# TrevorS/voxtral-mini-realtime-rs

Measured on NVIDIA H100. Metric: decode_tokens_per_sec, higher is better.
Workload: dtype f32

## Files before the change

voxtral_mini_realtime_rs_b200/csrc/capi.cu:

```cuda
#include <cuda_profiler_api.h>
#include <cuda_runtime.h>

#include <cstring>
#include <memory>
#include <string>
#include <vector>

#include "audio_host.h"
#include "common.h"
#include "gguf.h"
#include "kernels.h"
#include "model.h"
#include "stream.h"
#include "tokenizer.h"

namespace vox {
static thread_local std::string g_last_error;
void set_last_error(const std::string &m) { g_last_error = m; }
}

using namespace vox;

#define VOX_API_BEGIN try {
#define VOX_API_END                                \
// ... 882 lines not shown
    VOX_API_END
}
int32_t vox_session_nbest(vox_session *sh, int32_t *ids, double *scores, size_t cap, int32_t *b, int32_t *w, int32_t *n) {
    VOX_API_BEGIN
    REQUIRE(sh);
    Session *s = sh->s;
    s->sel.read_nbest(ids, scores, cap, b, w, n, s->st);
    VOX_API_END
}
int32_t vox_session_cache_len(const vox_session *s, int32_t *len) {
    VOX_API_BEGIN
    REQUIRE(s); REQUIRE(len);
    *len = s->s->cache_len;
    VOX_API_END
}
int32_t vox_session_reset(vox_session *s) {
    VOX_API_BEGIN
    REQUIRE(s);
    CUDA_OK(cudaSetDevice(s->s->m->device));
    s->s->reset();
    CUDA_OK(cudaStreamSynchronize(s->s->st));
    VOX_API_END
}
int32_t vox_session_debug_read(vox_session *sh, const char *what, float *out, size_t cap, size_t *n_floats) {
    VOX_API_BEGIN
    REQUIRE(sh); REQUIRE(what);
    Session *s = sh->s;
    const vox_model_info &c = s->m->info;
    CUDA_OK(cudaSetDevice(s->m->device));
    const std::string w = what;
    const float *src = nullptr;
    size_t n = 0;
    AudioEncoder &e = s->enc;
    const size_t rows = (size_t)e.rows;
    if (w == "capture_on" || w == "capture_off") {
        e.set_capture(*s, w == "capture_on");
        if (n_floats) *n_floats = 0;
        return VOX_OK;
    } else if (w == "graph_off" || w == "graph_on") {
        s->use_graph = (w == "graph_on");
        if (n_floats) *n_floats = 0;
        return VOX_OK;
    } else if (w == "enc_attn_simt" || w == "enc_attn_tc") {
        e.use_attn_tc = (w == "enc_attn_tc");
        if (n_floats) *n_floats = 0;
        return VOX_OK;
    } else if (w == "gemm_simt" || w == "gemm_tc") {
        s->path.gemm_tc = (w == "gemm_tc");
        if (n_floats) *n_floats = 0;
        return VOX_OK;
    } else if (w == "mega_off" || w == "mega_on" || w == "mega_auto") {
        s->use_mega = (w != "mega_off");
        if (n_floats) *n_floats = 0;
        return VOX_OK;
    } else if (w == "tc_off" || w == "tc_on") {
        s->path.matvec_tc = (w == "tc_on");
        if (n_floats) *n_floats = 0;
        return VOX_OK;
    } else if (w == "mega_epoch") {
        int epoch = 0;
        CUDA_OK(cudaStreamSynchronize(s->st));
        CUDA_OK(cudaMemcpy(&epoch, s->mega.epoch, sizeof(int), cudaMemcpyDeviceToHost));
        const float v[2] = {(float)s->mega.launches, (float)epoch};
        if (n_floats) *n_floats = 2;
        if (out) {
            VOX_CHECK(cap >= 2, VOX_ECAPACITY, "debug_read capacity %zu < 2", cap);
            memcpy(out, v, sizeof(v));
        }
        return VOX_OK;
    } else if (w == "mega_attn") {
        const size_t cnt = s->mega.attn_log.size() * 4;
        if (n_floats) *n_floats = cnt;
        if (out) {
            VOX_CHECK(cap >= cnt, VOX_ECAPACITY, "debug_read capacity %zu < %zu", cap, cnt);
            for (size_t i = 0; i < cnt; ++i) out[i] = (float)s->mega.attn_log[i / 4][i % 4];
        }
        return VOX_OK;
    } else if ((w.rfind("kv_k", 0) == 0 || w.rfind("kv_v", 0) == 0) && w.size() > 4) {
        const int l = atoi(w.c_str() + 4);
        VOX_CHECK(l >= 0 && l < c.dec_layers && std::to_string(l) == w.substr(4), VOX_EINVAL, "no decoder layer in '%s'", what);
        const int B = s->cur_B;
        std::vector<int> pos(B);
        CUDA_OK(cudaStreamSynchronize(s->st));
        if (B) CUDA_OK(cudaMemcpy(pos.data(), s->d_pos, sizeof(int) * B, cudaMemcpyDeviceToHost));
        const int L = B ? std::min(pos[0], s->kv.capacity()) : 0;
        for (int b = 0; b < B; ++b) VOX_CHECK(pos[b] == pos[0], VOX_EINVAL, "'%s': rows at different positions", what);
        const size_t cnt = (size_t)B * L * c.dec_kv_heads * c.dec_head_dim;
        if (n_floats) *n_floats = cnt;
        if (out && cnt) {
            VOX_CHECK(cap >= cnt, VOX_ECAPACITY, "debug_read capacity %zu < %zu", cap, cnt);
            s->kv.read(l, w[3] == 'v', B, L, out);
        }
        return VOX_OK;
    } else if (w == "mega_trace") {
        const size_t cnt = (size_t)s->mega.n_ops * 6;
        if (n_floats) *n_floats = cnt;
        if (out) {
            VOX_CHECK(cap >= cnt, VOX_ECAPACITY, "debug_read capacity %zu < %zu", cap, cnt);
            CUDA_OK(cudaStreamSynchronize(s->st));
            std::vector<unsigned long long> t(cnt);
            if (cnt) CUDA_OK(cudaMemcpy(t.data(), s->mega.trace, sizeof(unsigned long long) * cnt, cudaMemcpyDeviceToHost));
            int khz = 0;
            CUDA_OK(cudaDeviceGetAttribute(&khz, cudaDevAttrClockRate, s->m->device));
            for (size_t i = 0; i < cnt; ++i) out[i] = (float)((double)(t[i] - t[0]) / ((double)khz * 1e-3));
        }
        return VOX_OK;
// ... 299 lines not shown
```

voxtral_mini_realtime_rs_b200/csrc/decode_mega.cu:

```cuda
#include <cuda_fp16.h>

#include <cfloat>
#include <cmath>
#include <cstdlib>

#include "common.h"
#include "model.h"

namespace vox {

enum MegaKind : int {
    MG_EMBED = 0,
    MG_MATVEC = 1,
    MG_ATTN = 2,
    MG_ARGMAX = 3,
};

struct MegaOp {
    int kind = 0, epi = 0;
    const uint4 *qs_tc = nullptr;
    const uint2 *d_tc = nullptr;
    int N = 0, K = 0, n_tiles = 0, n_pairs = 0;
    int S = 1, Ps = 0;
    const uint2 *fin_bf = nullptr;
// ... 102 lines not shown
__host__ __device__ constexpr int mg_attn_fixed_bytes(int G, int HD) { return (G * HD + MG_CWARPS * G) * 4; }
__host__ __device__ constexpr int mg_attn_key_bytes(int G, int HD, KvType t) {
    return t == KvType::Q8 ? G * 4 + (2 * HD + 16) + 2 * (HD / KV_Q8_BLOCK) * 2
                           : G * 4 + (2 * HD + 16 / (t == KvType::F16 ? 2 : 4)) * (t == KvType::F16 ? 2 : 4);
}
__host__ __device__ constexpr int mg_attn_tile(int scratch_bytes, int G, int HD, KvType t) {
    return (scratch_bytes - mg_attn_fixed_bytes(G, HD)) / mg_attn_key_bytes(G, HD, t) / 32 * 32 > MG_CTHREADS
               ? MG_CTHREADS
               : (scratch_bytes - mg_attn_fixed_bytes(G, HD)) / mg_attn_key_bytes(G, HD, t) / 32 * 32;
}

__device__ __forceinline__ uint32_t smem_u32(const void *p) { return (uint32_t)__cvta_generic_to_shared(p); }
__device__ __forceinline__ void mbar_init(uint64_t *bar, uint32_t count) {
    asm volatile("mbarrier.init.shared::cta.b64 [%0], %1;\n" ::"r"(smem_u32(bar)), "r"(count));
}
__device__ __forceinline__ void mbar_expect_tx(uint64_t *bar, uint32_t bytes) {
    asm volatile("mbarrier.arrive.expect_tx.shared::cta.b64 _, [%0], %1;\n" ::"r"(smem_u32(bar)), "r"(bytes) : "memory");
}
__device__ __forceinline__ void mbar_arrive(uint64_t *bar) {
    asm volatile("mbarrier.arrive.shared::cta.b64 _, [%0];\n" ::"r"(smem_u32(bar)) : "memory");
}
__device__ __forceinline__ bool mbar_try(uint64_t *bar, uint32_t parity) {
    uint32_t ok;
    asm volatile(
        "{\n"
        ".reg .pred p;\n"
        "mbarrier.try_wait.parity.shared::cta.b64 p, [%1], %2;\n"
        "selp.u32 %0, 1, 0, p;\n"
        "}\n"
        : "=r"(ok)
        : "r"(smem_u32(bar)), "r"(parity)
        : "memory");
    return ok != 0;
}
__device__ __noinline__ void mg_die(unsigned *flag, unsigned code) {
    atomicExch(flag, code);
    __threadfence_system();
    __trap();
}
__device__ __forceinline__ void mbar_wait(uint64_t *bar, uint32_t parity, unsigned *flag, unsigned code) {
    if (mbar_try(bar, parity)) return;
    const long long t0 = clock64();
    unsigned n = 0;
    while (!mbar_try(bar, parity)) {
        if ((++n & 0x3FFFu) == 0 && clock64() - t0 > MG_SPIN_CYCLES) mg_die(flag, code);
    }
}
__device__ __forceinline__ void bulk_g2s(void *dst_smem, const void *src_gmem, uint32_t bytes, uint64_t *bar) {
    asm volatile("cp.async.bulk.shared::cluster.global.mbarrier::complete_tx::bytes [%0], [%1], %2, [%3];\n" ::"r"(
                     smem_u32(dst_smem)),
                 "l"(src_gmem), "r"(bytes), "r"(smem_u32(bar))
                 : "memory");
}
__device__ __forceinline__ unsigned ld_relaxed_u32(const unsigned *p) {
    unsigned v;
    asm volatile("ld.relaxed.gpu.global.u32 %0, [%1];\n" : "=r"(v) : "l"(p) : "memory");
    return v;
}
__device__ __forceinline__ void st_tagged(float2 *p, const float v, const int tag) {
    asm volatile("st.relaxed.gpu.global.v2.f32 [%0], {%1, %2};\n" ::"l"(p), "f"(v), "f"(__int_as_float(tag)) : "memory");
}
__device__ __forceinline__ float2 ld_tagged(const float2 *p) {
    float2 v;
    asm volatile("ld.relaxed.gpu.global.v2.f32 {%0, %1}, [%2];\n" : "=f"(v.x), "=f"(v.y) : "l"(p) : "memory");
    return v;
}
__device__ __forceinline__ void red_release_add(unsigned *p, unsigned v) {
    asm volatile("red.release.gpu.global.add.u32 [%0], %1;\n" ::"l"(p), "r"(v) : "memory");
}
__device__ __forceinline__ void cp_async16(void *dst_smem, const void *src_gmem) {
    asm volatile("cp.async.cg.shared.global [%0], [%1], 16;\n" ::"r"(smem_u32(dst_smem)), "l"(src_gmem) : "memory");
}
__device__ __forceinline__ void cp_async_commit() { asm volatile("cp.async.commit_group;\n" ::: "memory"); }
template <int N>
__device__ __forceinline__ void cp_async_wait() { asm volatile("cp.async.wait_group %0;\n" ::"n"(N) : "memory"); }
__device__ __forceinline__ void prefetch_l1(const void *p) { asm volatile("prefetch.global.L1 [%0];\n" ::"l"(p)); }
__device__ __forceinline__ void bulk_prefetch_l2(const void *p, uint32_t bytes) {
    asm volatile("cp.async.bulk.prefetch.L2.global [%0], %1;\n" ::"l"(p), "r"(bytes) : "memory");
}
__device__ __forceinline__ uint64_t policy_evict_first() {
    uint64_t pol;
    asm volatile("createpolicy.fractional.L2::evict_first.b64 %0, 1.0;\n" : "=l"(pol));
    return pol;
}
__device__ __forceinline__ void bulk_g2s_hint(void *dst_smem, const void *src_gmem, uint32_t bytes, uint64_t *bar, uint64_t pol) {
    asm volatile(
        "cp.async.bulk.shared::cluster.global.mbarrier::complete_tx::bytes.L2::cache_hint [%0], [%1], %2, [%3], %4;\n" ::"r"(
            smem_u32(dst_smem)),
        "l"(src_gmem), "r"(bytes), "r"(smem_u32(bar)), "l"(pol)
        : "memory");
}
__device__ __forceinline__ void cbar() { asm volatile("bar.sync 1, 512;\n" ::: "memory"); }
__device__ __forceinline__ void ebar() { asm volatile("bar.sync 2, %0;\n" ::"n"(MG_ETHREADS) : "memory"); }
__device__ __forceinline__ void abar() { asm volatile("bar.sync 3, %0;\n" ::"n"(MG_ATHREADS) : "memory"); }
__device__ __forceinline__ void hbar_arrive(const int id, const bool publish) {
    if (publish) asm volatile("fence.acq_rel.cta;\n" ::: "memory");
    asm volatile("bar.arrive %0, %1;\n" ::"r"(id), "n"(MG_ATHREADS) : "memory");
}
__device__ __forceinline__ void hbar_sync(const int id) { asm volatile("bar.sync %0, %1;\n" ::"r"(id), "n"(MG_ATHREADS) : "memory"); }

__device__ __forceinline__ void mma16816(float (&c)[4], const uint32_t a0, const uint32_t a1, const uint32_t a2,
                                         const uint32_t a3, const uint32_t b0, const uint32_t b1) {
    asm volatile(
        "mma.sync.aligned.m16n8k16.row.col.f32.f16.f16.f32 {%0,%1,%2,%3}, {%4,%5,%6,%7}, {%8,%9}, {%0,%1,%2,%3};\n"
        : "+f"(c[0]), "+f"(c[1]), "+f"(c[2]), "+f"(c[3])
        : "r"(a0), "r"(a1), "r"(a2), "r"(a3), "r"(b0), "r"(b1));
// ... 117 lines not shown
                blo[c] = make_uint2(0u, 0u);
                bhi[c] = blo[c];
                if (col < 2 * MT) {
                    blo[c] = bfb[col * 4 + t];
                    bhi[c] = bfb[(2 * MT + col) * 4 + t];
                }
                const int tok = c * 4 + t;
                of[c] = tok < MT ? ofp[bb * MT + tok] : make_float2(0.0f, 0.0f);
            }
#pragma unroll
            for (int u = 0; u < NTV; ++u) {
                const uint32_t wg = bb ? wq[u].z : wq[u].x, wg8 = bb ? wq[u].w : wq[u].y;
                const uint32_t dw = bb ? wd[u].y : wd[u].x;
                const float2 d = __half22float2(*reinterpret_cast<const __half2 *>(&dw));
                const uint32_t sg = wg >> 8, sg8 = wg8 >> 8;
#pragma unroll
                for (int c = 0; c < CG; ++c) {
                    float cc[4] = {0.f, 0.f, 0.f, 0.f};
                    mma16816(cc, wg & 0x000F000Fu, wg8 & 0x000F000Fu, sg & 0x000F000Fu, sg8 & 0x000F000Fu, blo[c].x, blo[c].y);
                    mma16816(cc, wg & 0x00F000F0u, wg8 & 0x00F000F0u, sg & 0x00F000F0u, sg8 & 0x00F000F0u, bhi[c].x, bhi[c].y);
                    acc[u][2 * c] = fmaf(d.x, fmaf(cc[0] + cc[1], of[c].y, of[c].x), acc[u][2 * c]);
                    acc[u][2 * c + 1] = fmaf(d.y, fmaf(cc[2] + cc[3], of[c].y, of[c].x), acc[u][2 * c + 1]);
                }
            }
        }
    }
}

template <int MT, int G, int DPL, bool RING, typename KV>
__global__ void __launch_bounds__(MG_THREADS, 1) decode_mega_kernel(const MegaParams p) {
    constexpr int CG = (MT + 3) / 4;
    constexpr int HD = DPL * 32;
    static_assert(G * HD <= MG_CTHREADS, "one attention output per consumer thread");
    constexpr int NT = mg_nt(MT);
    extern __shared__ __align__(128) unsigned char smem[];
    uint64_t *full = reinterpret_cast<uint64_t *>(smem);
    uint64_t *empty = full + MG_MAX_STAGES;
    float *rinv = reinterpret_cast<float *>(empty + MG_MAX_STAGES + 2);
    float *rpart = rinv + 8;
    uint64_t *stgc = reinterpret_cast<uint64_t *>(rpart + 32);
    float *red = reinterpret_cast<float *>(stgc + 4);
    float *acc_tile = red + 2 * MG_CWARPS * NT * 16 * MT;
    float *vals = acc_tile + MG_ACC_TILES * 16 * MT;
    MegaOp *s_op = reinterpret_cast<MegaOp *>(vals + mg_vals(MT));
    static_assert(sizeof(MegaOp) <= 256 && sizeof(MegaOp) % 4 == 0, "s_op");
    uint64_t *stg = empty + MG_MAX_STAGES;
    unsigned char *scratch = smem + mg_misc_bytes(MT);
    unsigned char *ring = scratch + p.scratch_bytes;
    const int tid = threadIdx.x, warp = tid >> 5, lane = tid & 31;
    const int g = lane >> 2, t = lane & 3;
    const int cta = blockIdx.x, nctas = gridDim.x;
    const int B = p.B, nstage = p.nstage;
    unsigned *wd_flag = p.bar + 2;

    if (tid == 0) {
        for (int i = 0; i < nstage; ++i) {
            mbar_init(&full[i], 1);
            mbar_init(&empty[i], MG_CWARPS);
        }
        mbar_init(stg, 1);
        for (int c = 0; c < 4; ++c) mbar_init(&stgc[c], 1);
        asm volatile("fence.mbarrier_init.release.cluster;\n" ::: "memory");
    }
    __syncthreads();

    if (warp >= MG_CWARPS) {
        asm volatile("setmaxnreg.dec.sync.aligned.u32 %0;\n" ::"n"(MG_REGS_PRODUCER));
        if (warp == MG_CWARPS && lane == 0) {
            int stage = 0;
            uint32_t phase = 0;
            bool wrapped = false;
            const uint64_t pol = policy_evict_first();
            for (int oi = 0; oi < p.n_ops; ++oi) {
                const MegaOp &op = p.ops[oi];
                if (oi + 1 < p.n_ops) {
                    const MegaOp &nx = p.ops[oi + 1];
                    const int who = (cta - oi % nctas + nctas) % nctas;
                    if (nx.kind == MG_MATVEC) {
                        if (nx.fout_ada_layer >= 0) {
                            if (who < B) bulk_prefetch_l2(p.ffn_ada_rows[who] + (size_t)nx.fout_ada_layer * p.D, (uint32_t)nx.N * 4u);
                        } else if (who == 0 && nx.fout_gamma) {
                            bulk_prefetch_l2(nx.fout_gamma, (uint32_t)nx.N * 4u);
                        }
                    }
                }
                if (op.kind != MG_MATVEC) continue;
                const int n_tiles = op.n_tiles, n_pairs = op.n_pairs, S = op.S, Ps = op.Ps, UT = op.unit_tiles;
                const uint4 *qs = op.qs_tc;
                const uint2 *ds = op.d_tc;
                const int ntl = mg_tile_count(n_tiles, UT, cta, nctas);
                for (int s = 0; s < S; ++s) {
                    const int pb = s * Ps;
                    const int np = min(Ps, n_pairs - pb);
                    for (int it = 0; it < ntl; it += NT) {
                        const int nt = min(NT, ntl - it);
                        for (int c0 = 0; c0 < np; c0 += MG_CHUNK) {
                            const int nb = min(MG_CHUNK, np - c0);
                            if (wrapped) mbar_wait(&empty[stage], phase ^ 1u, wd_flag, 0x100u + (unsigned)oi);
                            unsigned char *dst = ring + (size_t)stage * (NT * MG_SLOT_BYTES);
                            mbar_expect_tx(&full[stage], (uint32_t)(nt * nb) * 576u);
                            for (int u = 0; u < nt; ++u) {
                                const size_t pair0 = (size_t)mg_tile_of(it + u, UT, cta, nctas) * n_pairs + pb + c0;
                                bulk_g2s_hint(dst + (size_t)u * MG_SLOT_BYTES, qs + pair0 * 32, (uint32_t)nb * 512u, &full[stage], pol);
                                bulk_g2s_hint(dst + (size_t)u * MG_SLOT_BYTES + MG_SLOT_Q, ds + pair0 * 8, (uint32_t)nb * 64u, &full[stage], pol);
                            }
                            if (++stage == nstage) {
                                stage = 0;
                                phase ^= 1u;
                                wrapped = true;
                            }
                        }
                    }
                }
            }
        } else if (warp > MG_CWARPS) {
            constexpr int NOUT = NT * 16 * MT;
            constexpr int NQ = NOUT / 4;
// ... 290 lines not shown
                }
                if (oi + 1 < p.n_ops) {
                    abar();
                    abar();
                }
            }
        }
        return;
    }

    asm volatile("setmaxnreg.inc.sync.aligned.u32 %0;\n" ::"n"(MG_REGS_CONSUMER));
    const int epoch = *p.d_epoch;
    int stage = 0;
    uint32_t phase = 0, stg_phase = 0;
    int par = 0, group_ctr = 0;
    unsigned bar_target = 0;

    for (int oi = 0; oi < p.n_ops; ++oi) {
        const MegaOp &op = p.ops[oi];
        const int kind = op.kind;
        const bool tracing = p.trace != nullptr && cta == 0 && tid == 0;
        const bool tr_all = p.trace_all != nullptr && tid == 0;
        unsigned long long *const ta = tr_all ? p.trace_all + ((size_t)cta * p.n_ops + oi) * 4 : nullptr;
        if (tr_all) ta[0] = ta[3] = (unsigned long long)clock64();
        if (tracing) {
            const unsigned long long now = (unsigned long long)clock64();
            p.trace[oi * 6 + 0] = now;
            p.trace[oi * 6 + 1] = now;
            p.trace[oi * 6 + 4] = now;
            p.trace[oi * 6 + 5] = now;
        }
        if (tid == 0 && oi + 1 < p.n_ops) {
            prefetch_l1(&p.ops[oi + 1]);
            prefetch_l1(reinterpret_cast<const unsigned char *>(&p.ops[oi + 1]) + 128);
        }
        if (kind == MG_MATVEC) {
            const int n_tiles = op.n_tiles, n_pairs = op.n_pairs, S = op.S, Ps = op.Ps, K = op.K;
            const int UT = op.unit_tiles;
            const bool has_norm = op.gamma != nullptr;
            const int ntl = mg_tile_count(n_tiles, UT, cta, nctas);
            float2 *off2 = reinterpret_cast<float2 *>(scratch);
            uint2 *bf = reinterpret_cast<uint2 *>(off2 + (size_t)Ps * 2 * MT);
            if (ntl > 0) {
                for (int s = 0; s < S; ++s) {
                    const int pb = s * Ps;
                    const int np = min(Ps, n_pairs - pb);
                    const int CP = 16 * ((((np + 15) >> 4) + 3) >> 2);
                    cbar();
                    if (tid == 0) {
                        asm volatile("fence.proxy.async;\n" ::: "memory");
                        const uint32_t ob = (uint32_t)(2 * np * MT) * 8u;
                        const unsigned char *src = reinterpret_cast<const unsigned char *>(op.fin_bf + (size_t)(2 * pb) * (16 * MT));
                        unsigned char *dstb = reinterpret_cast<unsigned char *>(bf);
#pragma unroll
                        for (int c = 0; c < 4; ++c) {
                            const int p0 = min(np, c * CP), p1 = min(np, (c + 1) * CP);
                            const uint32_t o = (uint32_t)p0 * (256u * MT), cb = (uint32_t)(p1 - p0) * (256u * MT);
                            mbar_expect_tx(&stgc[c], cb + (c == 0 ? ob : 0u));
                            if (c == 0) bulk_g2s(off2, op.fin_off + (size_t)(2 * pb) * MT, ob, &stgc[0]);
                            if (cb) bulk_g2s(dstb + o, src + o, cb, &stgc[c]);
                        }
                    }
                    const uint32_t stg_par = stg_phase;
                    stg_phase ^= 1u;
                    if (s == 0 && has_norm && warp >= 1 && warp <= 4) {
                        const int total = op.ssq_in_parts * 8;
                        float pr[12];
#pragma unroll
                        for (int q = 0; q < 12; ++q) {
                            const int f = (warp - 1) * 32 + lane + 128 * q;
                            pr[q] = f < total ? __ldcg(op.ssq_in + f) : 0.0f;
                        }
                        float ss = 0.0f;
#pragma unroll
                        for (int q = 0; q < 12; ++q) ss += pr[q];
                        for (int f = (warp - 1) * 32 + lane + 128 * 12; f < total; f += 128) ss += __ldcg(op.ssq_in + f);
                        ss += __shfl_xor_sync(0xffffffffu, ss, 8);
                        ss += __shfl_xor_sync(0xffffffffu, ss, 16);
                        if (lane < 8) rpart[(warp - 1) * 8 + lane] = ss;
                    }
                    cbar();
                    if (s == 0 && has_norm && tid < B)
                        rinv[tid] = 1.0f / sqrtf((((rpart[tid] + rpart[8 + tid]) + (rpart[16 + tid] + rpart[24 + tid]))) / (float)K + p.eps);
                    if (tracing && s == 0) p.trace[oi * 6 + 1] = (unsigned long long)clock64();
                    for (int it = 0; it < ntl; it += NT) {
                        const int nt = min(NT, ntl - it);
                        float acc[NT][2 * CG];
#pragma unroll
                        for (int u = 0; u < NT; ++u)
#pragma unroll
                            for (int c = 0; c < 2 * CG; ++c) acc[u][c] = 0.0f;
                        {
                            const uint32_t slot_q = (uint32_t)warp * 512u + (uint32_t)lane * 16u;
                            const uint32_t slot_d = (uint32_t)MG_SLOT_Q + (uint32_t)warp * 64u + (uint32_t)g * 8u;
                            int next_chunk_c0 = it == 0 ? 0 : 0x7fffffff, chunk = 0;
                            for (int c0 = 0; c0 < np; c0 += MG_CHUNK) {
                                if (c0 == next_chunk_c0) {
                                    mbar_wait(&stgc[chunk], stg_par, wd_flag, 0x500u + (unsigned)oi);
                                    ++chunk;
                                    next_chunk_c0 += CP;
                                }
                                mbar_wait(&full[stage], phase, wd_flag, 0x200u + (unsigned)oi);
                                if (tracing && s == 0 && it == 0 && c0 == 0) p.trace[oi * 6 + 4] = (unsigned long long)clock64();
                                if (tr_all && s == 0 && it == 0 && c0 == 0) ta[3] = (unsigned long long)clock64();
                                const int pp = c0 + warp;
                                if (pp < np) {
                                    const unsigned char *sb = ring + (size_t)stage * (NT * MG_SLOT_BYTES);
                                    const uint2 *bfp = bf + (size_t)pp * (2 * 16 * MT);
                                    const float2 *ofp = off2 + (size_t)pp * (2 * MT);
                                    uint64_t *const rel = &empty[stage];
                                    if (nt == NT) mg_pair<MT, NT, NT>(sb, slot_q, slot_d, bfp, ofp, g, t, lane, acc, rel);
                                    else if (NT > 1 && nt == 1) mg_pair<MT, NT, 1>(sb, slot_q, slot_d, bfp, ofp, g, t, lane, acc, rel);
                                    else if (NT > 2 && nt == 2) mg_pair<MT, NT, 2>(sb, slot_q, slot_d, bfp, ofp, g, t, lane, acc, rel);
// ... 354 lines not shown
                if (warp < B) {
                    float bv = -INFINITY;
                    int bx = 0x7fffffff;
                    for (int c = lane; c < nctas; c += 32)
                        amax_combine(bv, bx, __ldcg(p.am_vals + (size_t)c * 8 + warp), __ldcg(p.am_idx + (size_t)c * 8 + warp));
#pragma unroll
                    for (int o = 16; o > 0; o >>= 1) {
                        const float ov = __shfl_xor_sync(0xffffffffu, bv, o);
                        const int ox = __shfl_xor_sync(0xffffffffu, bx, o);
                        amax_combine(bv, bx, ov, ox);
                    }
                    if (lane == 0) {
                        if (bx == 0x7fffffff) bx = 0;
                        p.d_tok[warp] = bx;
                        const int outpos = p.d_outpos[warp];
                        if (p.d_out) p.d_out[(size_t)warp * p.out_ld + outpos] = bx;
                        p.d_pos[warp] += 1;
                        p.d_outpos[warp] = outpos + 1;
                    }
                }
                if (tid == 0) *p.d_epoch = epoch + 1;
            }
        }
        if (tracing) p.trace[oi * 6 + 2] = (unsigned long long)clock64();
        if (tr_all) ta[1] = ta[2] = (unsigned long long)clock64();
        if (oi + 1 < p.n_ops) {
            abar();
            if (tid == 0) {
                red_release_add(&p.bar[0], 1u);
                bar_target += (unsigned)nctas;
                const long long t0 = clock64();
                unsigned n = 0;
                while (ld_relaxed_u32(&p.bar[0]) < bar_target) {
                    if ((++n & 0x3FFu) == 0 && clock64() - t0 > MG_SPIN_CYCLES) mg_die(wd_flag, 0x300u + (unsigned)oi);
                }
                asm volatile("fence.acq_rel.gpu;\n" ::: "memory");
            }
            abar();
            if (tracing) p.trace[oi * 6 + 3] = (unsigned long long)clock64();
            if (tr_all) ta[2] = (unsigned long long)clock64();
        }
    }
    if (tid == 0) {
        __threadfence();
        const unsigned old = atomicAdd(&p.bar[1], 1u);
        if (old == (unsigned)nctas - 1u) {
            p.bar[0] = 0u;
            p.bar[1] = 0u;
            __threadfence();
        }
    }
}

template <int MT, int G, int DPL, bool RING, typename KV>
void launch_t(const MegaParams &p, const MegaPlan &plan, int grid, cudaStream_t st) {
    static SmemAttr smem_attr;
    CUDA_OK(ensure_dyn_smem(decode_mega_kernel<MT, G, DPL, RING, KV>, MG_SMEM_MAX, smem_attr));
    cudaLaunchConfig_t cfg{};
    cfg.gridDim = dim3(grid);
    cfg.blockDim = dim3(MG_THREADS);
    cfg.dynamicSmemBytes = plan.smem_bytes;
    cfg.stream = st;
    cudaLaunchAttribute attr[1];
    attr[0].id = cudaLaunchAttributeCooperative;
    attr[0].val.cooperative = 1;
    cfg.attrs = attr;
    cfg.numAttrs = 1;
    CUDA_OK(cudaLaunchKernelEx(&cfg, decode_mega_kernel<MT, G, DPL, RING, KV>, p));
    tc_count_launch("decode_mega");
}

template <int MT, int G, int DPL>
void launch_g(const MegaParams &p, const MegaPlan &plan, int grid, cudaStream_t st) {
    if (plan.kv_type == KvType::Q8) (p.ring ? launch_t<MT, G, DPL, true, int8_t> : launch_t<MT, G, DPL, false, int8_t>)(p, plan, grid, st);
    else if (plan.kv_type == KvType::F16) (p.ring ? launch_t<MT, G, DPL, true, __half> : launch_t<MT, G, DPL, false, __half>)(p, plan, grid, st);
    else (p.ring ? launch_t<MT, G, DPL, true, float> : launch_t<MT, G, DPL, false, float>)(p, plan, grid, st);
}


using MegaLaunch = void (*)(const MegaParams &, const MegaPlan &, int, cudaStream_t);
template <int G, int DPL>
MegaLaunch mt_launch(int MT) {
    return MT == 1 ? launch_g<1, G, DPL> : MT == 2 ? launch_g<2, G, DPL> : MT == 4 ? launch_g<4, G, DPL>
                                                                             : launch_g<8, G, DPL>;
}
MegaLaunch find_launch(int MT, int H, int Hkv, int hd) {
    const int G = Hkv > 0 && H % Hkv == 0 ? H / Hkv : 0;
    if (G == 4 && hd == 128) return mt_launch<4, 4>(MT);
    if (G == 2 && hd == 32) return mt_launch<2, 1>(MT);
    return nullptr;
}

MegaPlan decode_mega_plan(int B, int max_pairs, int H, int Hkv, int hd, KvType kv_type) {
    MegaPlan pl;
    pl.kv_type = kv_type;
    pl.MT = B <= 1 ? 1 : (B <= 2 ? 2 : (B <= 4 ? 4 : 8));
    const int G = H / Hkv;
    const int attn_bytes = mg_attn_fixed_bytes(G, hd) + 32 * mg_attn_key_bytes(G, hd, kv_type);
    const int per_pair = mg_pair_bytes(pl.MT);
    int cap_pairs = MG_SCRATCH_CAP / per_pair;
    if (cap_pairs >= MG_CHUNK) cap_pairs = cap_pairs / MG_CHUNK * MG_CHUNK;
    pl.Ps_cap = max_pairs < cap_pairs ? max_pairs : cap_pairs;
    if (pl.Ps_cap < 1) pl.Ps_cap = 1;
    int scratch = pl.Ps_cap * per_pair;
    if (scratch < attn_bytes) scratch = attn_bytes;
    pl.scratch_bytes = (scratch + 127) & ~127;
    pl.attn_tile = mg_attn_tile(pl.scratch_bytes, G, hd, kv_type);
    const int left = MG_SMEM_MAX - mg_misc_bytes(pl.MT) - pl.scratch_bytes;
    const int stage_bytes = mg_nt(pl.MT) * MG_SLOT_BYTES;
    int ns = left / stage_bytes;
    pl.nstage = ns > MG_MAX_STAGES ? MG_MAX_STAGES : ns;
    VOX_CHECK(pl.nstage >= 2, VOX_EINVAL, "decode_mega: no room for the weight ring (%d stages)", pl.nstage);
    pl.smem_bytes = (size_t)mg_misc_bytes(pl.MT) + pl.scratch_bytes + (size_t)pl.nstage * stage_bytes;
    return pl;
}

}

struct MegaFrag {
    uint2 *bf = nullptr;
    float2 *off = nullptr;
    size_t blocks = 0;
};

struct DecodeMega::State {
    MegaParams p;
    MegaPlan plan;
    MegaOp *ops = nullptr;
    int ops_cap = 0;
    int rows = 0;
    int att_units = 0;
    size_t acc_floats = 0, ml_floats = 0;
    MegaFrag xf, af, cf;
    void clear_fragments(cudaStream_t st) const {
        for (const MegaFrag *f : {&xf, &af, &cf}) CUDA_OK(cudaMemsetAsync(f->bf, 0, sizeof(uint2) * f->blocks * 16 * MG_ROWS, st));
        for (const MegaFrag *f : {&xf, &af, &cf}) CUDA_OK(cudaMemsetAsync(f->off, 0, sizeof(float2) * f->blocks * MG_ROWS, st));
    }
};

DecodeMega::DecodeMega() : state(new State) {}
DecodeMega::~DecodeMega() = default;

void DecodeMega::create(Session &s) {
    const Model &m = *s.m;
    const vox_model_info &c = m.info;
    State &g = *state;
    MegaParams &p = g.p;
    CUDA_OK(cudaDeviceGetAttribute(&grid, cudaDevAttrMultiProcessorCount, m.device));
    g.ops_cap = 6 * c.dec_layers + 4;
    p.ops = g.ops = s.arena.alloc_n<MegaOp>(g.ops_cap);
    p.bar = s.arena.alloc_n<unsigned>(4);
    CUDA_OK(cudaMemset(p.bar, 0, sizeof(unsigned) * 4));
    p.am_vals = s.arena.alloc_n<float>((size_t)grid * MG_ROWS);
    p.am_idx = s.arena.alloc_n<int>((size_t)grid * MG_ROWS);
    g.att_units = std::max(grid, MG_ROWS * c.dec_kv_heads);
    const size_t units = g.att_units + MG_ROWS * c.dec_kv_heads, G = c.dec_heads / c.dec_kv_heads;
    g.acc_floats = 2 * units * G * c.dec_head_dim;
    g.ml_floats = 2 * units * G * 2;
    p.att_acc = s.arena.alloc_n<float>(g.acc_floats);
    p.att_ml = s.arena.alloc_n<float>(g.ml_floats);
    p.d_epoch = epoch = s.arena.alloc_n<int>(1);
    CUDA_OK(cudaMemset(p.att_acc, 0, sizeof(float) * g.acc_floats));
    CUDA_OK(cudaMemset(p.att_ml, 0, sizeof(float) * g.ml_floats));
    CUDA_OK(cudaMemset(epoch, 0, sizeof(int)));
    g.xf.blocks = 2 * mg_pairs(c.dec_dim);
    g.af.blocks = 2 * mg_pairs(c.dec_heads * c.dec_head_dim);
    g.cf.blocks = 2 * mg_pairs(c.dec_ffn);
    for (MegaFrag *f : {&g.xf, &g.af, &g.cf}) f->bf = s.arena.alloc_n<uint2>(f->blocks * 16 * MG_ROWS);
    for (MegaFrag *f : {&g.xf, &g.af, &g.cf}) f->off = s.arena.alloc_n<float2>(f->blocks * MG_ROWS);
    p.trace = trace = s.arena.alloc_n<unsigned long long>((size_t)g.ops_cap * 6);
    CUDA_OK(cudaMemset(trace, 0, sizeof(unsigned long long) * g.ops_cap * 6));
    if (const char *ta = getenv("VOX_MEGA_TRACE_ALL"); ta && ta[0] == '1') {
        const size_t n = (size_t)grid * g.ops_cap * 4;
        p.trace_all = trace_all = s.arena.alloc_n<unsigned long long>(n);
        CUDA_OK(cudaMemset(trace_all, 0, sizeof(unsigned long long) * n));
    }
    p.eps = m.norm_eps;
    p.qkv = s.qkv_dec;
    p.ld_qkv = (c.dec_heads + 2 * c.dec_kv_heads) * c.dec_head_dim;
    p.H = c.dec_heads;
    p.Hkv = c.dec_kv_heads;
    p.hd = c.dec_head_dim;
    const KvView kv = s.kv.view(0, s.d_pos);
    p.max_seq = kv.max_seq();
    p.page_table = kv.page_table;
    p.max_pages = kv.max_pages;
    p.window = c.dec_window;
    p.scale = powf((float)c.dec_head_dim, -0.5f);
    p.ring = kv.ring ? 1 : 0;
    p.attn_out = s.attn_dec;
    p.emb_qs = m.tok_emb.qs;
    p.emb_d = m.tok_emb.d;
    p.D = c.dec_dim;
    p.audio_off = s.d_audio_off;
    p.ffn_ada_rows = s.d_fga_rows;
    p.x_dec = s.x_dec;
    p.ssq_x = s.ssq_x;
    p.emb_fbf = g.xf.bf;
    p.emb_foff = g.xf.off;
    p.emb_gamma = m.dec[0].attn_norm;
    p.att_fbf = g.af.bf;
    p.att_foff = g.af.off;
    p.d_pos = s.d_pos;
    p.d_outpos = s.d_outpos;
    p.d_tok = s.d_tok;
    p.d_out = s.d_out;
    p.out_ld = s.out_ld;
}

unsigned DecodeMega::prepare(const Session &s, int R) {
    const Model &m = *s.m;
    const vox_model_info &c = m.info;
    State &g = *state;
    const int B = std::min(R, MG_ROWS);
    const unsigned groups = (unsigned)(R + MG_ROWS - 1) / MG_ROWS;
    const int D = c.dec_dim, H = c.dec_heads, Hkv = c.dec_kv_heads, hd = c.dec_head_dim;
    if (B < 1 || !find_launch(1, H, Hkv, hd)) return 0;
    if (g.rows == B) return n_ops > 0 ? groups : 0;
    g.rows = B;
    n_ops = 0;
    for (int j = 0; j < c.dec_layers; ++j)
        if (!m.dec[j].wqkv.qs_tc || !m.dec[j].wo.qs_tc || !m.dec[j].w13.qs_tc || !m.dec[j].w2.qs_tc) return 0;
    const int max_pairs = std::max(std::max(mg_pairs(D), mg_pairs(H * hd)), mg_pairs(c.dec_ffn));
    g.plan = decode_mega_plan(B, max_pairs, H, Hkv, hd, s.kv.type());
    const int parts = (D + 15) / 16;
    std::vector<MegaOp> ops;
    bool ok = true;
    auto matvec = [&](const Q4Weight &w, const MegaFrag &fin, float *y, int ldy, const float *res, int epi, const float *norm_w,
                      bool ssq_out_, bool track, int unit_tiles, const MegaFrag &fout, const float *fout_gamma) {
        MegaOp o;
        o.kind = MG_MATVEC;
        o.epi = epi;
        o.qs_tc = w.qs_tc;
        o.d_tc = w.d_tc;
        o.N = w.N;
        o.K = w.K;
        o.n_tiles = (w.N + 15) / 16;
        o.n_pairs = mg_pairs(w.K);
        int S = (o.n_pairs + g.plan.Ps_cap - 1) / g.plan.Ps_cap;
        int Ps = (o.n_pairs + S - 1) / S;
        if (S > 1) Ps = std::min(g.plan.Ps_cap, (Ps + 15) / 16 * 16);
        S = (o.n_pairs + Ps - 1) / Ps;
        o.S = S;
        o.Ps = Ps;
        o.unit_tiles = unit_tiles;
        if (o.n_tiles % unit_tiles != 0) ok = false;
        const int n_units = o.n_tiles / unit_tiles;
        if (S > 1 && ((n_units + grid - 1) / grid) * unit_tiles > MG_ACC_TILES) ok = false;
        o.fin_bf = fin.bf;
        o.fin_off = fin.off;
        o.fout_bf = fout.bf;
        o.fout_off = fout.off;
        o.fout_gamma = fout_gamma;
        o.y = y;
        o.ldy = ldy;
        o.res = res;
        o.gamma = norm_w;
        if (norm_w) {
            o.ssq_in = s.ssq_x;
            o.ssq_in_parts = parts;
        }
        if (ssq_out_) o.ssq_out = s.ssq_x;
        o.track_argmax = track ? 1 : 0;
        ops.push_back(o);
    };
    const MegaFrag none;
    {
        MegaOp e;
        e.kind = MG_EMBED;
        ops.push_back(e);
    }
    for (int j = 0; j < c.dec_layers; ++j) {
        const DecLayerW &l = m.dec[j];
        matvec(l.wqkv, g.xf, s.qkv_dec, g.p.ld_qkv, nullptr, EPI_NONE, l.attn_norm, false, false, 1, none, nullptr);
        const KvView kv = s.kv.view(j, s.d_pos);
        ops.back().kc = kv.k;
        ops.back().vc = kv.v;
        MegaOp a;
        a.kind = MG_ATTN;
        a.kc = kv.k;
        a.vc = kv.v;
        a.layer = j;
        ops.push_back(a);
        matvec(l.wo, g.af, s.x_dec, D, s.x_dec, EPI_RESIDUAL, nullptr, true, false, 2, g.xf, nullptr);
        ops.back().fout_ada_layer = j;
        matvec(l.w13, g.xf, nullptr, c.dec_ffn, nullptr, EPI_SILU_MUL, l.ffn_norm, false, false, 4, g.cf, nullptr);
        const float *next_norm = j + 1 < c.dec_layers ? m.dec[j + 1].attn_norm : m.dec_norm;
        matvec(l.w2, g.cf, s.x_dec, D, s.x_dec, EPI_RESIDUAL, nullptr, true, false, 2, g.xf, next_norm);
    }
    matvec(m.tok_emb, g.xf, s.logits, c.vocab, nullptr, EPI_NONE, m.dec_norm, false, true, 1, none, nullptr);
    {
        MegaOp f;
        f.kind = MG_ARGMAX;
        ops.push_back(f);
    }
    if (c.dec_ffn % 32 != 0 || (H * hd) % 32 != 0 || c.dec_layers > 63) ok = false;
    if ((D + 15) / 16 != parts || D % 32 != 0) ok = false;
    if (!ok || (int)ops.size() > g.ops_cap) return 0;
    g.clear_fragments(s.st);
    CUDA_OK(cudaMemcpyAsync(g.ops, ops.data(), sizeof(MegaOp) * ops.size(), cudaMemcpyHostToDevice, s.st));
    CUDA_OK(cudaStreamSynchronize(s.st));
    n_ops = g.p.n_ops = (int)ops.size();
    return groups;
}

void DecodeMega::step(const Session &s, int R, bool add_audio) {
    const State &g = *state;
    for (int b0 = 0; b0 < R; b0 += MG_ROWS) {
        const int B = std::min(MG_ROWS, R - b0);
        if (B < g.rows) {
            g.clear_fragments(s.st);
        }
        MegaParams p = g.p;
        p.B = B;
        p.page_table += (size_t)b0 * p.max_pages;
        p.audio_off += b0;
        p.ffn_ada_rows += b0;
        p.d_pos += b0;
        p.d_outpos += b0;
        p.d_tok += b0;
        p.d_out += (size_t)b0 * p.out_ld;
        p.audio = add_audio ? s.enc.audio : nullptr;
        p.logits_out = s.logits + (size_t)b0 * s.m->info.vocab;
        p.cos_t = s.dec_rope.cos_t;
        p.sin_t = s.dec_rope.sin_t;
        p.rope_rows = s.dec_rope.rows;
        p.attn_chunks = std::max(1, std::min(4, std::min(grid, g.att_units) / (B * p.Hkv)));
        p.nstage = g.plan.nstage;
        p.scratch_bytes = g.plan.scratch_bytes;
        attn_log.push_back({B, g.plan.MT, g.plan.attn_tile, p.attn_chunks});
        find_launch(g.plan.MT, p.H, p.Hkv, p.hd)(p, g.plan, grid, s.st);
        if (!capturing) ++launches;
    }
}

void DecodeMega::rebase_epoch(cudaStream_t st) {
    if (launches > (1u << 24)) {
        CUDA_OK(cudaMemsetAsync(state->p.att_acc, 0, sizeof(float) * state->acc_floats, st));
        CUDA_OK(cudaMemsetAsync(state->p.att_ml, 0, sizeof(float) * state->ml_floats, st));
        CUDA_OK(cudaMemsetAsync(epoch, 0, sizeof(int), st));
        launches = 0;
    }
}

}
```

voxtral_mini_realtime_rs_b200/csrc/decode_mega.h:

```cpp
#pragma once
#include <cuda_runtime.h>

#include <array>
#include <memory>
#include <vector>

namespace vox {

struct Session;

struct DecodeMega {
    DecodeMega();
    ~DecodeMega();
    void create(Session &s);
    unsigned prepare(const Session &s, int R);
    void step(const Session &s, int R, bool add_audio);
    void rebase_epoch(cudaStream_t st);

    unsigned launches = 0;
    bool capturing = false;
    std::vector<std::array<int, 4>> attn_log;
    int grid = 0, n_ops = 0;
    int *epoch = nullptr;
    unsigned long long *trace = nullptr, *trace_all = nullptr;

  private:
    struct State;
    std::unique_ptr<State> state;
};

}
```

voxtral_mini_realtime_rs_b200/csrc/model.cu:

```cuda
#include "model.h"

#include <algorithm>
#include <cmath>
#include <cstring>

#include "common.h"

namespace vox {

void cuda_check(cudaError_t e, const char *what) {
    if (e != cudaSuccess) fail(VOX_ECUDA, fmt("CUDA error: %s: %s", what, cudaGetErrorString(e)));
}

void *DeviceArena::alloc(size_t bytes) {
    if (bytes == 0) bytes = 16;
    void *p = nullptr;
    cudaError_t e = cudaMalloc(&p, bytes);
    if (e != cudaSuccess) fail(VOX_ENOMEM, fmt("cudaMalloc(%zu) failed: %s", bytes, cudaGetErrorString(e)));
    ptrs.push_back(p);
    total += bytes;
    return p;
}

void DeviceArena::release() {
// ... 597 lines not shown
                     fused_decode(B) ? ssq_x : nullptr, st);
        const bool pending = decoder_forward(B, 1);
        lm_head_rows(B, pending, logits);
        launch_argmax_multi(logits, B, m->info.vocab, d_tok, d_out, out_ld, d_outpos, am_vals, am_idx, am_cnt, st);
        launch_advance(d_pos, 1, d_outpos, 1, B, st);
    }
    sel.after_step(*this, B);
    return mega_launches;
}

void Session::set_bias(int stream, const int32_t *ids, const int32_t *lens, const float *boosts, int n) {
    if (sel.set_bias(stream, ids, lens, boosts, n, st)) bound_streams.clear();
}

void Session::prefill(int B, int M, const int *ids_host, bool add_audio) {
    const vox_model_info &c = m->info;
    bind_rows(B);
    CUDA_OK(cudaMemcpyAsync(d_ids, ids_host, sizeof(int) * (size_t)B * M, cudaMemcpyHostToDevice, st));
    launch_embed(m->tok_emb, d_ids, add_audio ? enc.audio : nullptr, d_audio_off, B, M, d_pos, x_dec,
                 fused_decode(B * M) ? ssq_x : nullptr, st);
    const bool pending = decoder_forward(B, M);
    if (pending) {
        launch_rmsnorm(x_dec, m->dec_norm, h_dec, B * M, c.dec_dim, m->norm_eps, st);
    }
    launch_gather_last(h_dec, last_h, B, M, c.dec_dim, st);
    linear(m->tok_emb, last_h, B, logits, c.vocab, nullptr, nullptr, EPI_NONE);
    launch_argmax(logits, B, c.vocab, d_tok, d_out, out_ld, d_outpos, st);
    launch_advance(d_pos, M, d_outpos, 1, B, st);
    sel.after_step(*this, B);
}

void Session::step_incremental(int b, int M, const int *ids_host, bool add_audio) {
    if (ids_host) prefill(b, M, ids_host, add_audio);
    else decode_step(b, add_audio);
    cache_len += M;
    sel.record_step(b, out_rows.data());
    for (int r = 0; r < b; ++r) ++out_rows[r];
}

void Session::reset() {
    CUDA_OK(cudaMemsetAsync(d_pos, 0, sizeof(int) * max_batch, st));
    CUDA_OK(cudaMemsetAsync(d_outpos, 0, sizeof(int) * max_batch, st));
    std::fill(out_rows.begin(), out_rows.end(), 0);
    cache_len = 0;
    kv.restore_identity(st);
    sel.clear_bias_history(-1, st);
    rebase_epoch();
}

template <class Step>
void Session::run_steps(int R, int n, Step step) {
    if (n <= 0) return;
    prepare_step(R);
    const StepKey key{R, sel.top_k, sel.beam_w, path.matvec_tc, path.gemm_tc, use_mega, sel.bias_on()};
    if (use_graph && !(step_graph.exec && step_graph.key == key)) {
        step();
        --n;
        if (step_graph.exec) { cudaGraphExecDestroy(step_graph.exec); step_graph.exec = nullptr; }
        if (n > 0) {
            cudaGraph_t graph = nullptr;
            const uint64_t before = kernel_launch_count();
            CUDA_OK(cudaStreamBeginCapture(st, cudaStreamCaptureModeThreadLocal));
            mega.capturing = true;
            try {
                step_graph.mega_launches = step();
            } catch (...) {
                mega.capturing = false;
                cudaStreamEndCapture(st, &graph);
                if (graph) cudaGraphDestroy(graph);
                throw;
            }
            mega.capturing = false;
            CUDA_OK(cudaStreamEndCapture(st, &graph));
            step_graph.nodes = kernel_launch_count() - before;
            add_graph_launches(-(int64_t)step_graph.nodes);
            cudaError_t e = cudaGraphInstantiate(&step_graph.exec, graph, 0);
            cudaGraphDestroy(graph);
            cuda_check(e, "cudaGraphInstantiate");
            step_graph.key = key;
        }
    }
    for (int i = 0; i < n; ++i) {
        if (!use_graph) { step(); continue; }
        CUDA_OK(cudaGraphLaunch(step_graph.exec, st));
        add_graph_launches((int64_t)step_graph.nodes);
        mega.launches += step_graph.mega_launches;
    }
}

namespace {
struct RowStreams {
    Session *s;
    ~RowStreams() { s->row_streams.clear(); }
};
}

int Session::transcribe_from_mel(int B, int T, int32_t *out_ids, size_t cap_ids, vox_timings *tm, bool total) {
    const vox_model_info &c = m->info;
    const int W = sel.beam_w, R = B * W;
    sel.check_rows(B);
    RowStreams row_guard{this};
    if (W > 1)
        for (int r = 0; r < R; ++r) row_streams.push_back(r % B);
    const std::vector<int> frames(B, T);
    enc.encode(*this, B, frames.data());
    cur_B = B;
    CUDA_OK(cudaEventRecord(ev[2], st));
// ... 143 lines not shown
```

voxtral_mini_realtime_rs_b200/csrc/model.h:

```cpp
#pragma once
#include <cuda_runtime.h>

#include <algorithm>
#include <cstdint>
#include <string>
#include <tuple>
#include <vector>

#include "audio_host.h"
#include "gguf.h"
#include "decode_mega.h"
#include "encoder.h"
#include "kernels.h"
#include "kv_cache.h"
#include "token_select.h"

namespace vox {

void cuda_check(cudaError_t e, const char *what);
#define CUDA_OK(x) ::vox::cuda_check((x), #x)

struct DeviceArena {
    int device = 0;
    std::vector<void *> ptrs;
// ... 15 lines not shown
void alloc_split_k(DeviceArena &arena, Work &w) {
    w.partial = arena.alloc_n<float>(w.partial_floats);
    w.counters = arena.alloc_n<int>(w.n_counters);
    CUDA_OK(cudaMemset(w.counters, 0, sizeof(int) * w.n_counters));
}

struct MelTables {
    float *window = nullptr;
    float *fb_vals = nullptr;
    int *fb_start = nullptr, *fb_len = nullptr;
    int fb_stride = 0;
    std::vector<float> fb_dense, window_host;
    void build(DeviceArena &arena);
};

struct EncLayerW {
    float *attn_norm = nullptr, *ffn_norm = nullptr;
    Q4Weight wqkv, wo, w13, w2;
    float *bqkv = nullptr, *bo = nullptr, *b2 = nullptr;
};
struct DecLayerW {
    float *attn_norm = nullptr, *ffn_norm = nullptr;
    Q4Weight ada0, ada2, wqkv, wo, w13, w2;
};

struct Model {
    int device = 0;
    vox_model_info info{};
    float rope_theta = 1e6f, norm_eps = 1e-5f;
    DeviceArena arena;
    float *conv1_w = nullptr, *conv1_b = nullptr, *conv2_w = nullptr, *conv2_b = nullptr;
    std::vector<EncLayerW> enc;
    float *enc_norm = nullptr;
    Q4Weight adapter0, adapter2, tok_emb;
    std::vector<DecLayerW> dec;
    float *dec_norm = nullptr;
    float *enc_cos = nullptr, *enc_sin = nullptr, *dec_cos = nullptr, *dec_sin = nullptr;
    int enc_rope_len = 4096, dec_rope_len = 16384;
    MelTables mel;
    RopeView dec_rope() const { return RopeView{dec_cos, dec_sin, dec_rope_len}; }

    static Model *load(const Gguf &g, int device);
};

void rope_rows(int hd, float theta, int64_t p0, int n, float *cos_out, float *sin_out);

Q4Weight upload_q4(DeviceArena &arena, const std::vector<const uint8_t *> &raw, const std::vector<int> &n_rows,
                   int K, bool interleave, bool tc_layout = false);

constexpr float kDefaultDelay = 6.0f;

struct StepKey {
    int rows = 0, top_k = 0, beam_w = 1;
    bool matvec_tc = true, gemm_tc = true, use_mega = true, bias = false;
    auto tie() const { return std::tie(rows, top_k, beam_w, matvec_tc, gemm_tc, use_mega, bias); }
    bool operator==(const StepKey &o) const { return tie() == o.tie(); }
};
struct StepGraph {
    StepKey key;
    cudaGraphExec_t exec = nullptr;
    uint64_t nodes = 0;
    unsigned mega_launches = 0;
};

struct Session {
    Model *m = nullptr;
    int max_batch = 0, M_max = 0;
    cudaStream_t st = nullptr;
    DeviceArena arena;
    cudaEvent_t ev[5] = {nullptr, nullptr, nullptr, nullptr, nullptr};
    AudioEncoder enc;
    int cur_B = 0;
    DecoderKv kv;
    RopeView dec_rope;
    float *x_dec = nullptr, *h_dec = nullptr, *qkv_dec = nullptr, *attn_dec = nullptr, *act_dec = nullptr;
    float *last_h = nullptr, *logits = nullptr;
    float *logits_all = nullptr;
    size_t logits_all_cap = 0;
    std::vector<float> delays;
    float *ada_sets = nullptr, *t_embed = nullptr, *ada_tmp = nullptr;
    size_t ada_set_floats() const { return (size_t)2 * m->info.dec_layers * m->info.dec_dim; }
    const float **d_ada_rows = nullptr, **d_fga_rows = nullptr;
    int64_t *d_audio_off = nullptr;
    std::vector<int> bound_streams;
    std::vector<int64_t> bound_offs;
    int *d_pos = nullptr, *d_outpos = nullptr, *d_tok = nullptr, *d_ids = nullptr, *d_out = nullptr;
    int out_ld = 0;
    int cache_len = 0;
    std::vector<int> row_streams;
    TokenSelect sel;
    void set_bias(int stream, const int32_t *ids, const int32_t *lens, const float *boosts, int n);
    std::vector<int> out_rows;
    StepGraph step_graph;
    bool use_graph = true;
    TcWork tc_split;
    float *ssq_x = nullptr;
    float *am_vals = nullptr;
    int *am_idx = nullptr, *am_cnt = nullptr;
    TcWork tc_work(bool norm_in, bool ssq_out) const;
    bool use_mega = true;
    DecodeMega mega;
    bool fused_decode(int rows) const;
    void *xt_buf = nullptr;
    size_t xt_elems = 0;
    GemmWork gemm_work;
    Q4Path path;

    static Session *create(Model *m, int max_batch, int max_mel_frames, bool kv_ring = false, KvType kv_type = KvType::F32);
// ... 27 lines not shown
```

Baseline: 3890.

## Launch decode megakernel in thread-block clusters with TMA multicast of activations

```diff
diff --git a/voxtral_mini_realtime_rs_b200/csrc/capi.cu b/voxtral_mini_realtime_rs_b200/csrc/capi.cu
--- a/voxtral_mini_realtime_rs_b200/csrc/capi.cu
+++ b/voxtral_mini_realtime_rs_b200/csrc/capi.cu
@@ -958,6 +958,17 @@
     } else if (w == "mega_off" || w == "mega_on" || w == "mega_auto") {
         s->use_mega = (w != "mega_off");
         if (n_floats) *n_floats = 0;
+        return VOX_OK;
+    } else if (w == "mega_cluster_1" || w == "mega_cluster_auto") {
+        s->mega.clusters = (w == "mega_cluster_auto");
+        if (n_floats) *n_floats = 0;
+        return VOX_OK;
+    } else if (w == "mega_cluster") {
+        if (n_floats) *n_floats = 1;
+        if (out) {
+            VOX_CHECK(cap >= 1, VOX_ECAPACITY, "debug_read capacity %zu < 1", cap);
+            out[0] = (float)s->mega.cluster;
+        }
         return VOX_OK;
     } else if (w == "tc_off" || w == "tc_on") {
         s->path.matvec_tc = (w == "tc_on");
diff --git a/voxtral_mini_realtime_rs_b200/csrc/decode_mega.cu b/voxtral_mini_realtime_rs_b200/csrc/decode_mega.cu
--- a/voxtral_mini_realtime_rs_b200/csrc/decode_mega.cu
+++ b/voxtral_mini_realtime_rs_b200/csrc/decode_mega.cu
@@ -178,6 +178,24 @@
                  "l"(src_gmem), "r"(bytes), "r"(smem_u32(bar))
                  : "memory");
 }
+__device__ __forceinline__ void bulk_g2s_multicast(void *dst_smem, const void *src_gmem, uint32_t bytes, uint64_t *bar,
+                                                   uint16_t mask) {
+    asm volatile(
+        "cp.async.bulk.shared::cluster.global.mbarrier::complete_tx::bytes.multicast::cluster [%0], [%1], %2, [%3], %4;\n" ::"r"(
+            smem_u32(dst_smem)),
+        "l"(src_gmem), "r"(bytes), "r"(smem_u32(bar)), "h"(mask)
+        : "memory");
+}
+__device__ __forceinline__ uint32_t cluster_rank() {
+    uint32_t r;
+    asm volatile("mov.u32 %0, %%cluster_ctarank;\n" : "=r"(r));
+    return r;
+}
+__device__ __forceinline__ uint32_t cluster_size() {
+    uint32_t n;
+    asm volatile("mov.u32 %0, %%cluster_nctarank;\n" : "=r"(n));
+    return n;
+}
 __device__ __forceinline__ unsigned ld_relaxed_u32(const unsigned *p) {
     unsigned v;
     asm volatile("ld.relaxed.gpu.global.u32 %0, [%1];\n" : "=r"(v) : "l"(p) : "memory");
@@ -401,6 +419,7 @@
     const int cta = blockIdx.x, nctas = gridDim.x;
     const int B = p.B, nstage = p.nstage;
     unsigned *wd_flag = p.bar + 2;
+    const uint32_t ncl = cluster_size();
 
     if (tid == 0) {
         for (int i = 0; i < nstage; ++i) {
@@ -412,6 +431,7 @@
         asm volatile("fence.mbarrier_init.release.cluster;\n" ::: "memory");
     }
     __syncthreads();
+    if (ncl > 1) asm volatile("barrier.cluster.arrive.release.aligned;\nbarrier.cluster.wait.acquire.aligned;\n" ::: "memory");
 
     if (warp >= MG_CWARPS) {
         asm volatile("setmaxnreg.dec.sync.aligned.u32 %0;\n" ::"n"(MG_REGS_PRODUCER));
@@ -808,13 +828,20 @@
                         const uint32_t ob = (uint32_t)(2 * np * MT) * 8u;
                         const unsigned char *src = reinterpret_cast<const unsigned char *>(op.fin_bf + (size_t)(2 * pb) * (16 * MT));
                         unsigned char *dstb = reinterpret_cast<unsigned char *>(bf);
+                        const uint32_t ncl = s == 0 ? cluster_size() : 1u, crank = ncl > 1 ? cluster_rank() : 0u;
 #pragma unroll
                         for (int c = 0; c < 4; ++c) {
                             const int p0 = min(np, c * CP), p1 = min(np, (c + 1) * CP);
                             const uint32_t o = (uint32_t)p0 * (256u * MT), cb = (uint32_t)(p1 - p0) * (256u * MT);
                             mbar_expect_tx(&stgc[c], cb + (c == 0 ? ob : 0u));
-                            if (c == 0) bulk_g2s(off2, op.fin_off + (size_t)(2 * pb) * MT, ob, &stgc[0]);
-                            if (cb) bulk_g2s(dstb + o, src + o, cb, &stgc[c]);
+                            if (ncl == 1) {
+                                if (c == 0) bulk_g2s(off2, op.fin_off + (size_t)(2 * pb) * MT, ob, &stgc[0]);
+                                if (cb) bulk_g2s(dstb + o, src + o, cb, &stgc[c]);
+                            } else if ((uint32_t)c % ncl == crank) {
+                                const uint16_t mask = (uint16_t)((1u << ncl) - 1u);
+                                if (c == 0) bulk_g2s_multicast(off2, op.fin_off + (size_t)(2 * pb) * MT, ob, &stgc[0], mask);
+                                if (cb) bulk_g2s_multicast(dstb + o, src + o, cb, &stgc[c], mask);
+                            }
                         }
                     }
                     const uint32_t stg_par = stg_phase;
@@ -1275,8 +1302,25 @@
     }
 }
 
+int mega_cluster_size(const void *kernel, cudaLaunchConfig_t cfg, int grid) {
+    for (const int n : {4, 2}) {
+        if (grid % n != 0) continue;
+        cudaLaunchAttribute a;
+        a.id = cudaLaunchAttributeClusterDimension;
+        a.val.clusterDim.x = (unsigned)n;
+        a.val.clusterDim.y = 1;
+        a.val.clusterDim.z = 1;
+        cfg.attrs = &a;
+        cfg.numAttrs = 1;
+        int clusters = 0;
+        CUDA_OK(cudaOccupancyMaxActiveClusters(&clusters, kernel, &cfg));
+        if (clusters * n >= grid) return n;
+    }
+    return 1;
+}
+
 template <int MT, int G, int DPL, bool RING, typename KV>
-void launch_t(const MegaParams &p, const MegaPlan &plan, int grid, cudaStream_t st) {
+int launch_t(const MegaParams &p, const MegaPlan &plan, int grid, int cluster, cudaStream_t st) {
     static SmemAttr smem_attr;
     CUDA_OK(ensure_dyn_smem(decode_mega_kernel<MT, G, DPL, RING, KV>, MG_SMEM_MAX, smem_attr));
     cudaLaunchConfig_t cfg{};
@@ -1284,24 +1328,30 @@
     cfg.blockDim = dim3(MG_THREADS);
     cfg.dynamicSmemBytes = plan.smem_bytes;
     cfg.stream = st;
-    cudaLaunchAttribute attr[1];
+    if (cluster == 0) return mega_cluster_size(reinterpret_cast<const void *>(decode_mega_kernel<MT, G, DPL, RING, KV>), cfg, grid);
+    cudaLaunchAttribute attr[2];
     attr[0].id = cudaLaunchAttributeCooperative;
     attr[0].val.cooperative = 1;
+    attr[1].id = cudaLaunchAttributeClusterDimension;
+    attr[1].val.clusterDim.x = (unsigned)cluster;
+    attr[1].val.clusterDim.y = 1;
+    attr[1].val.clusterDim.z = 1;
     cfg.attrs = attr;
-    cfg.numAttrs = 1;
+    cfg.numAttrs = cluster > 1 ? 2 : 1;
     CUDA_OK(cudaLaunchKernelEx(&cfg, decode_mega_kernel<MT, G, DPL, RING, KV>, p));
     tc_count_launch("decode_mega");
+    return cluster;
 }
 
 template <int MT, int G, int DPL>
-void launch_g(const MegaParams &p, const MegaPlan &plan, int grid, cudaStream_t st) {
-    if (plan.kv_type == KvType::Q8) (p.ring ? launch_t<MT, G, DPL, true, int8_t> : launch_t<MT, G, DPL, false, int8_t>)(p, plan, grid, st);
-    else if (plan.kv_type == KvType::F16) (p.ring ? launch_t<MT, G, DPL, true, __half> : launch_t<MT, G, DPL, false, __half>)(p, plan, grid, st);
-    else (p.ring ? launch_t<MT, G, DPL, true, float> : launch_t<MT, G, DPL, false, float>)(p, plan, grid, st);
-}
-
-
-using MegaLaunch = void (*)(const MegaParams &, const MegaPlan &, int, cudaStream_t);
+int launch_g(const MegaParams &p, const MegaPlan &plan, int grid, int cluster, cudaStream_t st) {
+    if (plan.kv_type == KvType::Q8) return (p.ring ? launch_t<MT, G, DPL, true, int8_t> : launch_t<MT, G, DPL, false, int8_t>)(p, plan, grid, cluster, st);
+    if (plan.kv_type == KvType::F16) return (p.ring ? launch_t<MT, G, DPL, true, __half> : launch_t<MT, G, DPL, false, __half>)(p, plan, grid, cluster, st);
+    return (p.ring ? launch_t<MT, G, DPL, true, float> : launch_t<MT, G, DPL, false, float>)(p, plan, grid, cluster, st);
+}
+
+
+using MegaLaunch = int (*)(const MegaParams &, const MegaPlan &, int, int, cudaStream_t);
 template <int G, int DPL>
 MegaLaunch mt_launch(int MT) {
     return MT == 1 ? launch_g<1, G, DPL> : MT == 2 ? launch_g<2, G, DPL> : MT == 4 ? launch_g<4, G, DPL>
@@ -1349,6 +1399,7 @@
 struct DecodeMega::State {
     MegaParams p;
     MegaPlan plan;
+    int cluster = 1;
     MegaOp *ops = nullptr;
     int ops_cap = 0;
     int rows = 0;
@@ -1446,6 +1497,7 @@
         if (!m.dec[j].wqkv.qs_tc || !m.dec[j].wo.qs_tc || !m.dec[j].w13.qs_tc || !m.dec[j].w2.qs_tc) return 0;
     const int max_pairs = std::max(std::max(mg_pairs(D), mg_pairs(H * hd)), mg_pairs(c.dec_ffn));
     g.plan = decode_mega_plan(B, max_pairs, H, Hkv, hd, s.kv.type());
+    g.cluster = find_launch(g.plan.MT, H, Hkv, hd)(g.p, g.plan, grid, 0, s.st);
     const int parts = (D + 15) / 16;
     std::vector<MegaOp> ops;
     bool ok = true;
@@ -1520,6 +1572,10 @@
     if (c.dec_ffn % 32 != 0 || (H * hd) % 32 != 0 || c.dec_layers > 63) ok = false;
     if ((D + 15) / 16 != parts || D % 32 != 0) ok = false;
     if (!ok || (int)ops.size() > g.ops_cap) return 0;
+    for (const MegaOp &o : ops) {
+        const int units = o.kind == MG_MATVEC ? o.n_tiles / o.unit_tiles : grid;
+        while (g.cluster > 1 && units < grid && units % g.cluster != 0) g.cluster /= 2;
+    }
     g.clear_fragments(s.st);
     CUDA_OK(cudaMemcpyAsync(g.ops, ops.data(), sizeof(MegaOp) * ops.size(), cudaMemcpyHostToDevice, s.st));
     CUDA_OK(cudaStreamSynchronize(s.st));
@@ -1552,7 +1608,7 @@
         p.nstage = g.plan.nstage;
         p.scratch_bytes = g.plan.scratch_bytes;
         attn_log.push_back({B, g.plan.MT, g.plan.attn_tile, p.attn_chunks});
-        find_launch(g.plan.MT, p.H, p.Hkv, p.hd)(p, g.plan, grid, s.st);
+        cluster = find_launch(g.plan.MT, p.H, p.Hkv, p.hd)(p, g.plan, grid, clusters ? g.cluster : 1, s.st);
         if (!capturing) ++launches;
     }
 }
diff --git a/voxtral_mini_realtime_rs_b200/csrc/decode_mega.h b/voxtral_mini_realtime_rs_b200/csrc/decode_mega.h
--- a/voxtral_mini_realtime_rs_b200/csrc/decode_mega.h
+++ b/voxtral_mini_realtime_rs_b200/csrc/decode_mega.h
@@ -19,6 +19,8 @@
 
     unsigned launches = 0;
     bool capturing = false;
+    bool clusters = true;
+    int cluster = 0;
     std::vector<std::array<int, 4>> attn_log;
     int grid = 0, n_ops = 0;
     int *epoch = nullptr;
diff --git a/voxtral_mini_realtime_rs_b200/csrc/model.cu b/voxtral_mini_realtime_rs_b200/csrc/model.cu
--- a/voxtral_mini_realtime_rs_b200/csrc/model.cu
+++ b/voxtral_mini_realtime_rs_b200/csrc/model.cu
@@ -673,7 +673,7 @@
 void Session::run_steps(int R, int n, Step step) {
     if (n <= 0) return;
     prepare_step(R);
-    const StepKey key{R, sel.top_k, sel.beam_w, path.matvec_tc, path.gemm_tc, use_mega, sel.bias_on()};
+    const StepKey key{R, sel.top_k, sel.beam_w, path.matvec_tc, path.gemm_tc, use_mega, sel.bias_on(), mega.clusters};
     if (use_graph && !(step_graph.exec && step_graph.key == key)) {
         step();
         --n;
diff --git a/voxtral_mini_realtime_rs_b200/csrc/model.h b/voxtral_mini_realtime_rs_b200/csrc/model.h
--- a/voxtral_mini_realtime_rs_b200/csrc/model.h
+++ b/voxtral_mini_realtime_rs_b200/csrc/model.h
@@ -91,8 +91,8 @@
 
 struct StepKey {
     int rows = 0, top_k = 0, beam_w = 1;
-    bool matvec_tc = true, gemm_tc = true, use_mega = true, bias = false;
-    auto tie() const { return std::tie(rows, top_k, beam_w, matvec_tc, gemm_tc, use_mega, bias); }
+    bool matvec_tc = true, gemm_tc = true, use_mega = true, bias = false, mega_clusters = true;
+    auto tie() const { return std::tie(rows, top_k, beam_w, matvec_tc, gemm_tc, use_mega, bias, mega_clusters); }
     bool operator==(const StepKey &o) const { return tie() == o.tie(); }
 };
 struct StepGraph {
```

Result: no change. 3866 (median of 6 runs) (-0.6%).
